# m4drat/wtf

Hardware: AMD Instinct MI355X
Metric: execs/sec + emulated instr/s per node (tlv_server, HEVD) at 1/2/4/8 GPUs (higher is better)
Workload: dtype u64

## Files before the change

### wtf_amd/csrc/engine_run.h

```cpp
#pragma once
#include <hip/hip_runtime.h>

#include "engine_fast.h"

using namespace wtfgpu_dev;

namespace {

__device__ __forceinline__ u64 wave_sum(u64 v) {
#pragma unroll
  for (int off = 32; off > 0; off >>= 1) v += __shfl_xor(v, off, 64);
  return v;
}
__device__ __forceinline__ u64 readlane64(u64 v, int l) {
  const u32 lo = __builtin_amdgcn_readlane((u32)v, l);
  const u32 hi = __builtin_amdgcn_readlane((u32)(v >> 32), l);
  return ((u64)hi << 32) | lo;
}
__device__ __forceinline__ u64 m_eq32(u32 a, u32 b) { return __builtin_amdgcn_uicmp(a, b, 32); }
__device__ __forceinline__ u64 m_ne32(u32 a, u32 b) { return __builtin_amdgcn_uicmp(a, b, 33); }
__device__ __forceinline__ u64 m_eq64(u64 a, u64 b) { return __builtin_amdgcn_uicmpl(a, b, 32); }
__device__ __forceinline__ u64 m_ne64(u64 a, u64 b) { return __builtin_amdgcn_uicmpl(a, b, 33); }
__device__ __forceinline__ u64 m_lt64(u64 a, u64 b) { return __builtin_amdgcn_uicmpl(a, b, 36); }
__device__ __forceinline__ u64 m_ge64(u64 a, u64 b) { return __builtin_amdgcn_uicmpl(a, b, 35); }
__device__ __forceinline__ u64 m_ge32(u32 a, u32 b) { return __builtin_amdgcn_uicmp(a, b, 35); }
__device__ __forceinline__ bool in_mask(u64 m) { return __builtin_amdgcn_inverse_ballot_w64(m); }

__device__ __forceinline__ bool hash_find(const u64 *keys, u32 mask, u64 key, u32 &slot) {
  u32 h = (u32)mix64(key) & mask;
  for (u32 i = 0; i <= mask; i++) {
    const u64 k = rfl64(keys[h]);
    if (k == key) {
      slot = h;
      return true;
    }
    if (k == EMPTY_KEY) return false;
    h = (h + 1) & mask;
  }
  return false;
}

__device__ __forceinline__ bool set_has(const u64 *keys, u32 mask, u64 key) {
  u32 h = (u32)mix64(key) & mask;
  for (u32 i = 0; i <= mask; i++) {
    const u64 k = keys[h];
    if (k == key) return true;
    if (k == EMPTY_KEY) return false;
    h = (h + 1) & mask;
  }
  return false;
}

__device__ __forceinline__ void trace_rip(const Dev &P, u32 lane, u64 rip) {
  const u32 n = P.trace_cnt[lane];
  if (n < P.trace_cap) P.trace[(u64)lane * P.trace_cap + n] = rip;
  P.trace_cnt[lane] = n + 1;
}

__device__ __forceinline__ u64 edge_key(u64 rip, u64 next) {
  u64 e = rip;
  e ^= e >> 30;
  e *= 0xbf58476d1ce4e5b9ull;
  e ^= e >> 27;
  e *= 0x94d049bb133111ebull;
  e ^= e >> 31;
  return e ^ next;
}

__device__ __forceinline__ bool edge_op(u32 op, u32 bsrc) {
  return op == O_JCC || op == O_LOOP || ((op == O_JMP || op == O_CALL) && bsrc != L_IMM);
}

__device__ __forceinline__ void load_lane(const Dev &P, u32 lane, Lane &L) {
  const u64 N = P.nlanes;
#pragma unroll
  for (int i = 0; i < 16; i++) RS(L, i, P.gpr[i * N + lane]);
  L.rip = P.rip[lane];
  L.rflags = P.rflags[lane];
  L.icount = P.icount[lane];
  L.nbytes = P.nbytes[lane];
  L.status = P.status[lane];
  const LaneSys s = P.sys[lane];
  L.cr0 = s.cr0;
  L.cr3 = s.cr3;
  L.efer = s.efer;
  L.cpl = s.cpl;
  L.simd = simd_bits(s.cr0, s.cr4, P.full[lane].xcr0);
  L.ovn = P.ov_count[lane];
  L.lane = lane;
  L.cgen = P.lane_gen ? P.lane_gen[lane] : 0;
  L.ccnt = P.cov_cnt ? P.cov_cnt[lane] : 0;
  if (P.tlb_ok && P.tlb_ok[lane]) {
    const LaneTlb &t = P.tlbs[lane];
#pragma unroll
    for (int i = 0; i < TLB_N; i++) {
      L.tv[i] = t.tv[i];
      L.td[i] = t.td[i];
    }
    L.cvpn = t.cvpn;
    L.cptr = t.cptr;
    L.bloom = t.bloom;
    L.tnext = t.tnext;
  } else {
    L.bloom = 0;
    for (u32 k = 0; k < L.ovn; k++) L.bloom |= bloom_bit(P.ov_gpfn[(u64)k * N + lane]);
    tlb_flush(L);
    L.tnext = 0;
  }
  L.exvec = L.exerr = L.exop = 0;
  L.exaddr = 0;
  L.miss = L.miss_acc = L.flush = L.pend = 0;
  L.nodeliver = 0;
  L.miss_va = 0;
}

__device__ __forceinline__ void store_tlb(const Dev &P, const Lane &L) {
  if (!P.tlb_ok) return;
  LaneTlb &t = P.tlbs[L.lane];
#pragma unroll
  for (int i = 0; i < TLB_N; i++) {
    t.tv[i] = L.tv[i];
    t.td[i] = L.td[i];
  }
  t.cvpn = L.cvpn;
  t.cptr = L.cptr;
  t.bloom = L.bloom;
  t.tnext = L.tnext;
  P.tlb_ok[L.lane] = 1;
}
__device__ __forceinline__ void tlb_stale(const Dev &P, u32 lane) {
  if (P.tlb_ok) P.tlb_ok[lane] = 0;
}

__device__ __forceinline__ void store_lane(const Dev &P, const Lane &L) {
  const u64 N = P.nlanes;
  const u32 lane = L.lane;
#pragma unroll
  for (int i = 0; i < 16; i++) P.gpr[i * N + lane] = R(L, i);
  P.rip[lane] = L.rip;
  P.rflags[lane] = L.rflags;
  P.icount[lane] = L.icount;
  P.nbytes[lane] = L.nbytes;
  P.status[lane] = L.status;
  P.ov_count[lane] = L.ovn;
  if (P.cov_cnt) P.cov_cnt[lane] = L.ccnt;
}

__device__ __forceinline__ u32 log_value(const Dev &P, u64 v, bool mine, u32 lane, u32 gen, u32 cnt);

__device__ __noinline__ u32 cover(const Dev &P, u64 rip, bool mine, u32 lane, u32 gen, u32 cnt) {
  if (P.code_keys) {
    u32 s;
    if (hash_find(P.code_keys, P.code_mask, rip >> 12, s)) {
      const u32 cs = rfl32(P.code_slot[s]);
      if (rfl32(P.cov_map[(u64)cs * WTFGPU_PAGE_SIZE + (rip & 0xfff)])) return cnt;
    } else if (P.extra_keys && set_has(P.extra_keys, P.extra_mask, rip)) {
      return cnt;
    }
  }
  return log_value(P, rip, mine, lane, gen, cnt);
}

__device__ __forceinline__ void count_edge(const Dev &P, u32 lane, bool fresh) {
  if (!P.edge_cnt) return;
  P.edge_cnt[2 * (u64)lane] += 1;
  if (fresh) P.edge_cnt[2 * (u64)lane + 1] += 1;
}

__device__ __noinline__ u32 cover_edge(const Dev &P, u64 e, bool mine, u32 lane, u32 gen, u32 cnt) {
  if (!mine) return cnt;
  if (P.extra_keys && set_has(P.extra_keys, P.extra_mask, e)) return cnt;
  return log_value(P, e, true, lane, gen, cnt);
}

__device__ __forceinline__ u32 log_value(const Dev &P, u64 rip, bool mine, u32 lane, u32 gen, u32 cnt) {
  if (!mine) return cnt;
  const u32 H = P.H;
  const u64 base = (u64)lane * H;
  u32 h = (u32)mix64(rip) & (H - 1);
  for (u32 probe = 0; probe < H; probe++) {
    const u64 idx = base + h;
    if (P.cov_gen[idx] != gen) {
      if (cnt >= H - H / 4) {
        P.cov_overflow[lane] = 1;
        return cnt;
      }
      P.cov_rip[idx] = rip;
      P.cov_gen[idx] = gen;
      return cnt + 1;
    }
    if (P.cov_rip[idx] == rip) return cnt;
    h = (h + 1) & (H - 1);
  }
  return cnt;
}

__device__ __forceinline__ void fetch_bytes(u64 pageptr, u32 off, u32 n, u64 &lo, u64 &hi) {
  const u64 a = (pageptr + off) & ~7ull;
  const u32 sh = (u32)((pageptr + off) & 7);
  const u64 pend = pageptr + WTFGPU_PAGE_SIZE;
  const u64 w0 = rfl64(*(const u64 *)a);
  const u64 w1 = (a + 8 < pend) ? rfl64(*(const u64 *)(a + 8)) : 0;
  const u64 w2 = (a + 16 < pend) ? rfl64(*(const u64 *)(a + 16)) : 0;
  if (sh == 0) {
    lo = w0;
    hi = w1;
  } else {
    lo = (w0 >> (8 * sh)) | (w1 << (64 - 8 * sh));
    hi = (w1 >> (8 * sh)) | (w2 << (64 - 8 * sh));
  }
  if (n < 16) {
    if (n <= 8) {
      hi = 0;
      lo = n == 8 ? lo : (lo & ((1ull << (8 * n)) - 1));
    } else {
      hi &= (1ull << (8 * (n - 8))) - 1;
    }
  }
}

constexpr u32 UC_N = 312;
constexpr u32 UC_U = 4;
constexpr u32 UC_BP = 1, UC_COVERED = 2, UC_CROSS = 4, UC_BADLEN = 8, UC_UNSUP = 16;
struct UCHead {
  u64 key;
  u64 logged;
  u32 flags, pad;
  FOp f;
};
struct UCEntry {
  union {
    UCHead h;
    struct {
      u64 key;
      u64 logged;
      u32 flags, pad;
      FOp f;
    };
  };
  u64 rip;
};
struct UCUop {
  u64 key;
  UOp u;
};
struct GPayload {
  u32 flags, pad;
  FOp f;
  UOp u;
};
constexpr u32 GP_HEAD = (sizeof(u32) * 2 + sizeof(FOp)) / 4;
static_assert(sizeof(UOp) % 4 == 0 && sizeof(FOp) % 4 == 0, "copied as dwords");
static_assert(sizeof(UCEntry) == 64, "LDS entry size");
constexpr u32 UC_QUEUES = 2;
constexpr u64 UC_IMAGE_BYTES = (u64)UC_N * sizeof(UCEntry);

constexpr u32 UC_WAYS = 2;
static_assert(UC_N % UC_WAYS == 0, "whole sets");
__device__ __forceinline__ bool cacheable_key(u64 lptr, u64 pool_lo, u64 pool_span) {
  return !m_ge64(lptr - pool_lo, pool_span);
}
__device__ __forceinline__ u32 uc_slot(u64 key) {
  const u32 h = ((u32)key ^ (u32)(key >> 17)) * 0x9E3779B1u;
  return __umulhi(h, UC_N / UC_WAYS) * UC_WAYS;
}
__device__ __forceinline__ u32 uu_slot(u64 key) { return (u32)((key ^ (key >> 12) * 0x9E3779B1u) & (UC_U - 1)); }

template <typename T>
__device__ __forceinline__ void lds_uniform_read(const T *src, T &dst) {
  const u32 *s = (const u32 *)src;
  u32 *d = (u32 *)&dst;
#pragma unroll
  for (u32 i = 0; i < sizeof(T) / 4; i++) d[i] = rfl32(s[i]);
}

__device__ __forceinline__ void uc_head_read(const UCEntry *e, UCHead &h) {
  h.key = rfl64(e->key);
  h.flags = rfl32(e->flags);
  h.f.w0 = rfl32(e->f.w0);
  h.f.fl = rfl32(e->f.fl);
  h.f.w2 = rfl32(e->f.w2);
  h.f.disp = rfl64(e->f.disp);
  h.f.imm = rfl64(e->f.imm);
}

__device__ __forceinline__ bool bp_lookup(const Dev &P, u64 rip) {
  u32 s;
  return P.bp_keys && hash_find(P.bp_keys, P.bp_mask, rip, s);
}

__device__ __forceinline__ bool lane_phys_write(const Dev &P, Lane &L, u64 gpa, const u8 *src, u64 len) {
  while (len) {
    const u64 off = gpa & 0xfff;
    u64 n = 4096 - off;
    if (n > len) n = len;
    bool priv;
    const u8 *pg = phys_page(P, L.lane, L.ovn, L.bloom, gpa >> 12, priv);
    u8 *dst = (u8 *)pg;
    if (!priv) {
      if (L.ovn >= P.K) return false;
      dst = cow_copy(P, L.lane, L.ovn, gpa >> 12, pg);
      L.ovn++;
      L.bloom |= bloom_bit(gpa >> 12);
    }
    for (u64 i = 0; i < n; i++) dst[off + i] = src[i];
    src += n;
    gpa += n;
    len -= n;
  }
  return true;
}

__device__ __forceinline__ bool lane_phys_write64(const Dev &P, Lane &L, u64 gpa, u64 v) {
  bool priv;
  const u8 *pg = phys_page(P, L.lane, L.ovn, L.bloom, gpa >> 12, priv);
  u8 *dst = (u8 *)pg;
  if (!priv) {
    if (L.ovn >= P.K) return false;
    dst = cow_copy(P, L.lane, L.ovn, gpa >> 12, pg);
    L.ovn++;
    L.bloom |= bloom_bit(gpa >> 12);
  }
  *(u64 *)(dst + (gpa & 0xfff)) = v;
  return true;
}

__device__ __forceinline__ bool has_error_code(u32 vec) {
  return vec == 8 || (vec >= 10 && vec <= 14) || vec == 17 || vec == 21 || vec == 29 || vec == 30;
}
__device__ __forceinline__ bool sup_xlate(const Dev &P, Lane &L, u64 va, int acc, u64 &gpa) {
  u64 td, gpfn;
  if (!walk(P, L, va, acc, td, gpfn)) return false;
  gpa = (gpfn << 12) | (va & 0xfff);
  return true;
}
__device__ __noinline__ bool deliver_fault(const Dev &P, Lane &L) {
  LaneSys &S = P.sys[L.lane];
  const u32 vec = L.exvec, err = L.exerr;
  const u64 cr2 = L.exaddr, frip = L.rip;
  const u32 st0 = L.status, cpl0 = L.cpl;
  bool ok = false;
  do {
    if (S.deliv_icount == L.icount) break;
    if (!S.idtr || vec > 31 || (u64)vec * 16 + 15 > S.idtr_limit) break;
    u64 ga;
    if (!sup_xlate(P, L, S.idtr + vec * 16, ACC_R, ga) || (ga & 0xfff) > 4096 - 16) break;
    bool priv;
    const u8 *g = phys_page(P, L.lane, L.ovn, L.bloom, ga >> 12, priv) + (ga & 0xfff);
    const u64 lo = *(const u64 *)g, hi = *(const u64 *)(g + 8);
    const u32 attr = (u32)(lo >> 40) & 0xff, type = attr & 0xf, ist = (u32)(lo >> 32) & 7;
    if (!(attr & 0x80) || (type != 0xe && type != 0xf)) break;
    const u64 target = (lo & 0xffff) | ((lo >> 32) & 0xffff0000ull) | (hi << 32);
    const u16 sel = (u16)((lo >> 16) & 0xffff);
    const u32 ncpl = sel & 3;
    if (!canonical(target) || ncpl > L.cpl) break;
    u64 rsp = R(L, 4);
    if (ist || ncpl < L.cpl) {
      const u64 off = ist ? 0x24 + (u64)(ist - 1) * 8 : 4 + (u64)ncpl * 8;
      u64 ta;
      if (!sup_xlate(P, L, S.tss + off, ACC_R, ta) || (ta & 0xfff) > 4096 - 8) break;
      const u8 *t = phys_page(P, L.lane, L.ovn, L.bloom, ta >> 12, priv) + (ta & 0xfff);
      u64 v = 0;
      for (int i = 0; i < 8; i++) v |= (u64)t[i] << (8 * i);
      rsp = v;
    }
    rsp &= ~0xfull;
    const bool ec = has_error_code(vec);
    const u32 n = ec ? 6 : 5;
    const u64 ors = R(L, 4), orfl = L.rflags, ocs = S.cs, oss = S.ss;
    L.cpl = 0;
    bool wr = true;
    for (u32 i = 0; i < n && wr; i++) {
      const u32 k = ec ? i : i + 1;
      const u64 w = k == 0 ? (u64)err : k == 1 ? frip : k == 2 ? ocs : k == 3 ? orfl : k == 4 ? ors : oss;
      u64 pa;
      wr = sup_xlate(P, L, rsp - 8 * n + 8 * i, ACC_W, pa) && (pa & 7) == 0 && lane_phys_write64(P, L, pa, w);
    }
    if (!wr) break;
    if (ncpl < cpl0) S.ss = (u16)ncpl;
    set_cs(L, S, sel);
    if (vec == WTFGPU_VEC_PF) S.cr2 = cr2;
    L.cpl = S.cpl = ncpl;
    S.deliv_icount = L.icount;
    RS(L, 4, rsp - 8 * n);
    L.rflags &= ~(0x100ull | 0x4000ull | 0x10000ull | 0x20000ull | (type == 0xe ? 0x200ull : 0));
    L.rip = target;
    L.status = WTFGPU_RUNNING;
    tlb_flush(L);
    L.flush = 0;
    ok = true;
  } while (0);
  if (!ok) {
    L.cpl = cpl0;
    L.status = st0;
    L.exvec = vec;
    L.exerr = err;
    L.exaddr = cr2;
    L.nodeliver = 1;
  }
  return ok;
}

constexpr u32 GUC_WORDS = 48;
constexpr u32 GUC_PAYLOAD = sizeof(GPayload) / 4;
static_assert(GUC_PAYLOAD <= 3 * 14, "global uop cache entry: 3 lines of 14 payload dwords");
__device__ __forceinline__ u32 guc_slot(const Dev &P, u64 key) {
  return (u32)(mix64(key) & P.guc_mask);
}
__device__ __forceinline__ u32 guc_payload_index(u32 lid) {
  return (lid < GUC_WORDS && (lid & 15) < 14) ? (lid >> 4) * 14 + (lid & 15) : ~0u;
}

__device__ __forceinline__ u32 covered_flag(const Dev &P, u64 rip, u32 off) {
  if (P.code_keys) {
    u32 s;
    if (hash_find(P.code_keys, P.code_mask, rip >> 12, s)) {
      const u32 cs = rfl32(P.code_slot[s]);
      if (rfl32(P.cov_map[(u64)cs * WTFGPU_PAGE_SIZE + off])) return UC_COVERED;
    }
  }
  return 0;
}

__device__ __forceinline__ u32 covered_flag_lane(const Dev &P, u64 rip, u32 off) {
  if (!P.code_keys) return 0;
  u32 h = (u32)mix64(rip >> 12) & P.code_mask;
  for (u32 i = 0; i <= P.code_mask; i++) {
    const u64 k = P.code_keys[h];
    if (k == (rip >> 12)) return P.cov_map[(u64)P.code_slot[h] * WTFGPU_PAGE_SIZE + off] ? UC_COVERED : 0;
    if (k == EMPTY_KEY) return 0;
    h = (h + 1) & P.code_mask;
  }
  return 0;
}

__device__ __forceinline__ FOp generic_fop(const UOp &d) {
  FOp f{};
  f.w0 = (d.len & 0x3f) << 20;
  return f;
}

__device__ __forceinline__ bool uc_fill_shared(const Dev &P, UCEntry *e, UCUop *us, u64 key, u32 off, u64 rip,
                                               u32 lid) {
  if (!P.guc) return false;
  const u32 pj = guc_payload_index(lid);
  u32 *head = e ? (u32 *)&e->flags : nullptr, *uop = us ? (u32 *)&us->u : nullptr;
  u32 *gw = P.guc + (u64)guc_slot(P, key) * GUC_WORDS;
  const u32 w = lid < GUC_WORDS ? gw[lid] : 0;
  const bool tag = lid < GUC_WORDS && (lid & 15) >= 14;
  const bool bad = tag && w != ((lid & 1) ? (u32)(key >> 32) : (u32)key);
  if (__ballot(bad) != 0) return false;
  if (pj < GP_HEAD) {
    if (head) head[pj] = w;
  } else if (pj < GUC_PAYLOAD) {
    if (uop) uop[pj - GP_HEAD] = w;
  }
  const u32 sflags = __builtin_amdgcn_readlane(w, 0);
  u32 flags = sflags;
  if (e && !(sflags & UC_COVERED)) {
    flags |= covered_flag(P, rip, off);
    if ((flags & UC_COVERED) && lid == 0) gw[0] = flags;
  }
  __builtin_amdgcn_wave_barrier();
  if (lid == 0) {
    if (us) us->key = key;
    if (e) {
      e->logged = 0;
      e->flags = flags;
      e->rip = rip;
      e->key = key;
    }
  }
  return true;
}

__device__ __noinline__ void uc_fill(const Dev &P, UCEntry *e, UCUop *us, u64 key, u64 lptr, u32 off, u64 rip,
                                     u32 lid, bool shared_checked = false) {
  const u32 pj = guc_payload_index(lid);
  u32 *uop = (u32 *)&us->u;
  if (!shared_checked && uc_fill_shared(P, e, us, key, off, rip, lid)) return;
  u32 *gw = P.guc ? P.guc + (u64)guc_slot(P, key) * GUC_WORDS : nullptr;
  IBytes ib;
  ib.avail = 4096 - off < 16 ? 4096 - off : 16;
  fetch_bytes(lptr, off, ib.avail, ib.lo, ib.hi);
  UOp d;
  const int dr = decode(ib, d);
  u32 flags = dr == 1 ? UC_CROSS : dr == 2 ? UC_BADLEN : 0;
  FOp f;
  if (dr == 0) {
    digest(d, f);
    if (P.edges && edge_op(d.op, d.bsrc)) f = generic_fop(d);
    if (P.trace || g_tn.buf) f = generic_fop(d);
    if (!d.supported) flags |= UC_UNSUP;
    if (bp_lookup(P, rip)) flags |= UC_BP;
  } else {
    f = FOp{};
  }
  const u32 dyn = (dr == 0 && e) ? covered_flag(P, rip, off) : 0;
  if (lid == 0) {
    us->u = d;
    us->key = key;
  }
  __builtin_amdgcn_wave_barrier();
  __builtin_amdgcn_fence(__ATOMIC_RELEASE, "wavefront");
  if (gw) {
    u32 v = 0;
    if (pj < GP_HEAD) v = pj == 0 ? (flags | dyn) : pj == 1 ? 0u : ((const u32 *)&f)[pj - 2];
    else if (pj < GUC_PAYLOAD) v = uop[pj - GP_HEAD];
    else if (lid < GUC_WORDS && (lid & 15) >= 14) v = (lid & 1) ? (u32)(key >> 32) : (u32)key;
    if (lid < GUC_WORDS) gw[lid] = v;
  }
  if (lid == 0 && e) {
    e->logged = 0;
    e->f = f;
    e->flags = flags | dyn;
    e->rip = rip;
    e->key = key;
  }
}

__device__ __forceinline__ const UOp *uc_uop(const Dev &P, UCUop *uu, u64 key, u64 lptr, u32 off, u64 rip, u32 lid) {
  UCUop *us = &uu[uu_slot(key)];
  if (rfl64(us->key) != key) uc_fill(P, nullptr, us, key, lptr, off, rip, lid);
  return &us->u;
}

__device__ __noinline__ void code_xlate(const Dev &P, Lane &L, u64 rip) {
  u64 td;
  const u64 vpn = rip >> 12;
  if (!tlb_get(L, vpn, td) || !perm_ok(L, td, ACC_X)) {
    if (service_miss(P, L, rip & ~0xfffull, ACC_X)) tlb_get(L, vpn, td);
    else td = 0;
    if (td && !perm_ok(L, td, ACC_X)) td = 0;
    if (!td && L.status == WTFGPU_EXIT_FAULT) L.exaddr = rip;
  }
  if (td) {
    L.cvpn = vpn;
    L.cptr = (td & ~0xfffull) | (L.efer & EFER_M32);
  }
}

__device__ __noinline__ bool miss_service(const Dev &P, Lane &L, int attempt) {
  if (attempt >= 16 || !service_miss(P, L, L.miss_va, (int)L.miss_acc)) {
    if (attempt >= 16) set_fault(L, WTFGPU_VEC_GP, 0xffff, L.miss_va);
    return false;
  }
  return true;
}

__device__ __noinline__ int exec_generic(const Dev &P, Lane &L, const UOp *ul, u64 &next) {
  UOp d;
  lds_uniform_read(ul, d);
  return exec(P, L, d, L.rip + d.len, next);
}

__device__ __noinline__ int exec_retry(const Dev &P, Lane &L, const UOp *ul, u64 &next) {
  int x;
  tn_insn_begin(L.lane);
  for (int attempt = 0;; attempt++) {
    L.miss = 0;
    L.pend = 0;
    tn_rollback(L.lane);
    x = exec_generic(P, L, ul, next);
    if (!L.miss || L.status != WTFGPU_RUNNING) break;
    if (!miss_service(P, L, attempt)) break;
  }
  return x;
}

__device__ __forceinline__ void retire(const Dev &P, Lane &L, int x, u32 len, u64 next, u32 opbytes) {
  if (L.flush) {
    tlb_flush(L);
    L.flush = 0;
  }
  if ((x == X_OK || x == X_CR3) && L.status == WTFGPU_RUNNING) {
    L.rip = next;
    L.icount++;
    L.nbytes += len + L.pend;
    if (P.limit && L.icount > P.limit) L.status = WTFGPU_EXIT_TIMEOUT;
    else if (x == X_CR3) L.status = WTFGPU_EXIT_CR3;
  } else if (L.status != WTFGPU_RUNNING) {
  } else if (x == X_UNIMPL) {
    L.status = WTFGPU_EXIT_UNIMPLEMENTED;
    L.exop = len >= 4 ? opbytes : (opbytes & ((1u << (8 * len)) - 1));
  } else if (x == X_INT3) {
    L.status = WTFGPU_EXIT_INT3;
  } else if (x == X_HLT) {
    L.status = WTFGPU_EXIT_HLT;
  }
}

__device__ __noinline__ bool host_write(const Dev &P, Lane &L, u64 va, const u8 *__restrict__ src, u64 n) {
  const u32 cpl0 = L.cpl;
  const u64 cr00 = L.cr0;
  L.cpl = 0;
  L.cr0 &= ~(1ull << 16);
  bool ok = true;
  for (u64 o = 0; o < n;) {
    const u64 a = va + o, room = 4096 - (a & 0xfff);
    const u32 m = (u32)(n - o < room ? n - o : room);
    u8 *d = nullptr;
    u64 td = 0;
    for (int attempt = 0;; attempt++) {
      L.miss = 0;
      if ((d = xlate(L, a, ACC_W, &td))) break;
      if (L.status != WTFGPU_RUNNING || !L.miss || !miss_service(P, L, attempt)) {
        ok = false;
        break;
      }
    }
    if (!ok) break;
    if (td & T_PT) L.flush = 1;
    const u8 *__restrict__ sp = src + o;
    u32 k = 0;
    for (; k + 32 <= m; k += 32) {
      u8 t[32];
#pragma unroll
      for (u32 j = 0; j < 32; j++) t[j] = sp[k + j];
#pragma unroll
      for (u32 j = 0; j < 32; j++) d[k + j] = t[j];
    }
    for (; k < m; k++) d[k] = sp[k];
    o += m;
  }
  if (!ok) {
    if (L.status == WTFGPU_RUNNING || L.status == WTFGPU_EXIT_FAULT) L.status = WTFGPU_EXIT_FEED_FAULT;
    L.miss = 0;
  }
  L.cpl = cpl0;
  L.cr0 = cr00;
  L.pend = 0;
  if (ok && L.flush) {
    tlb_flush(L);
    L.flush = 0;
  }
  return ok;
}

__device__ __noinline__ bool feed_apply(const Dev &P, Lane &L, const wtfgpu_bp_action_t &a) {
  if (!P.feed_pos) return false;
  const u64 pos = P.feed_pos[L.lane];
  if (pos == ~0ull) return false;
  const u64 end = P.feed_end[L.lane];
  if (pos + 4 > end) {
    L.status = WTFGPU_EXIT_STOP_OK;
    return true;
  }
  const u8 *src = P.feed_data + pos;
  const u32 n = (u32)src[0] | ((u32)src[1] << 8) | ((u32)src[2] << 16) | ((u32)src[3] << 24);
  P.feed_pos[L.lane] = pos + 4 + n;
  if (n >= a.value || pos + 4 + n > end) {
    L.status = WTFGPU_EXIT_STOP_OK;
    return true;
  }
  const u32 rb = (u32)a.gprs[0] & 15, rn = (u32)a.gprs[1] & 15;
  const u64 dst = R(L, rb) + a.value - n;
  if (!host_write(P, L, dst, src + 4, n)) return true;
  RS(L, rn, n);
  RS(L, rb, dst);
  return true;
}

__device__ __noinline__ void insert_apply(const Dev &P, Lane &L, const wtfgpu_insert_t &ins) {
  const u64 pos = P.feed_pos[L.lane], end = P.feed_end[L.lane];
  if (pos == ~0ull) return;
  P.feed_pos[L.lane] = end;
  if (pos + 8 > end) return;
  const u8 *src = P.feed_data + pos;
  const u32 n = (u32)src[0] | ((u32)src[1] << 8) | ((u32)src[2] << 16) | ((u32)src[3] << 24);
  if (n < 4 || pos + 4 + n > end) return;
  const u32 head = (u32)src[4] | ((u32)src[5] << 8) | ((u32)src[6] << 16) | ((u32)src[7] << 24);
  const u64 m = n - 4;
  RS(L, ins.head_reg & 15, head);
  if (!host_write(P, L, R(L, ins.ptr_reg & 15), src + 8, m)) return;
  RS(L, ins.len_reg & 15, m);
  if (ins.len_arg) {
    u8 le[8];
    for (int i = 0; i < 8; i++) le[i] = (u8)(m >> (8 * i));
    host_write(P, L, R(L, WTFGPU_RSP) + 8 + 8 * (u64)ins.len_arg, le, 8);
  }
}

__device__ __forceinline__ u32 rotr32(u32 x, u32 n) { return (x >> n) | (x << (32 - n)); }
__device__ __forceinline__ void b3_g(u32 *v, int a, int b, int c, int d, u32 x, u32 y) {
  v[a] = v[a] + v[b] + x;
  v[d] = rotr32(v[d] ^ v[a], 16);
  v[c] = v[c] + v[d];
  v[b] = rotr32(v[b] ^ v[c], 12);
  v[a] = v[a] + v[b] + y;
  v[d] = rotr32(v[d] ^ v[a], 8);
  v[c] = v[c] + v[d];
  v[b] = rotr32(v[b] ^ v[c], 7);
}
__device__ __noinline__ void blake3_le64(u64 in, u64 &lo, u64 &hi) {
  const u32 iv[8] = {0x6A09E667u, 0xBB67AE85u, 0x3C6EF372u, 0xA54FF53Au,
                     0x510E527Fu, 0x9B05688Cu, 0x1F83D9ABu, 0x5BE0CD19u};
  const u8 perm[16] = {2, 6, 3, 10, 7, 0, 4, 13, 1, 11, 12, 5, 9, 14, 15, 8};
  u32 m[16] = {(u32)in, (u32)(in >> 32), 0, 0, 0, 0, 0, 0, 0, 0, 0, 0, 0, 0, 0, 0};
  u32 v[16] = {iv[0], iv[1], iv[2], iv[3], iv[4], iv[5], iv[6], iv[7], iv[0], iv[1], iv[2], iv[3], 0, 0, 8, 1 | 2 | 8};
  for (int r = 0; r < 7; r++) {
    b3_g(v, 0, 4, 8, 12, m[0], m[1]);
    b3_g(v, 1, 5, 9, 13, m[2], m[3]);
    b3_g(v, 2, 6, 10, 14, m[4], m[5]);
    b3_g(v, 3, 7, 11, 15, m[6], m[7]);
    b3_g(v, 0, 5, 10, 15, m[8], m[9]);
    b3_g(v, 1, 6, 11, 12, m[10], m[11]);
    b3_g(v, 2, 7, 8, 13, m[12], m[13]);
    b3_g(v, 3, 4, 9, 14, m[14], m[15]);
    if (r < 6) {
      u32 t[16];
      for (int i = 0; i < 16; i++) t[i] = m[perm[i]];
      for (int i = 0; i < 16; i++) m[i] = t[i];
    }
  }
  lo = (u64)(v[0] ^ v[8]) | ((u64)(v[1] ^ v[9]) << 32);
  hi = (u64)(v[2] ^ v[10]) | ((u64)(v[3] ^ v[11]) << 32);
}

__device__ __forceinline__ bool bp_apply_action(const Dev &P, Lane &L, u64 grip, const wtfgpu_bp_action_t *found) {
  u32 s;
  if (!found && (!P.act_keys || !hash_find(P.act_keys, P.act_mask, grip, s))) return false;
  const wtfgpu_bp_action_t &a = found ? *found : P.act[s];
  if (a.kind == WTFGPU_BPACT_SET_GPRS) {
    for (u32 i = 0; i < 16; i++) RS(L, i, a.gprs[i]);
    L.rip = a.gprs[16];
    return true;
  }
  if (a.kind == WTFGPU_BPACT_FEED) return feed_apply(P, L, a);
  if (a.kind == WTFGPU_BPACT_STOP_OK) {
    L.status = WTFGPU_EXIT_STOP_OK;
    return true;
  }
  if (a.kind == WTFGPU_BPACT_RDRAND) {
    if (!P.rd_seed) return false;
    u64 lo, hi;
    blake3_le64(P.rd_seed[L.lane], lo, hi);
    P.rd_seed[L.lane] = lo;
    RS(L, (u32)a.gprs[0] & 15, hi);
    return true;
  }
  if (a.kind == WTFGPU_BPACT_STOP_ARGS) {
    if (!P.stop_args) return false;
    const u64 rsp = R(L, WTFGPU_RSP);
    u64 v[6] = {R(L, 1), R(L, 2), R(L, 8), R(L, 9), 0, 0};
    for (u32 i = 4; i < 6 && i < a.value; i++) {
      for (int attempt = 0;; attempt++) {
        L.miss = 0;
        if (vread(L, rsp + 8 + 8 * (u64)i, 8, v[i])) break;
        if (L.status != WTFGPU_RUNNING || !L.miss || !miss_service(P, L, attempt)) {
          L.status = WTFGPU_RUNNING;
          L.miss = 0;
          L.pend = 0;
          return false;
        }
      }
    }
    L.pend = 0;
    for (u32 i = 0; i < 6; i++) P.stop_args[(u64)L.lane * 6 + i] = i < a.value ? v[i] : 0;
    L.status = WTFGPU_EXIT_STOP_ARGS;
    return true;
  }
  if (a.kind != WTFGPU_BPACT_RETURN) return false;
  if (a.gprs[0]) {
    const u64 s = R(L, (u32)(a.gprs[0] - 1) & 15);
    const u64 lim = a.gprs[1];
    for (u64 i = 0; i < lim;) {
      const u64 va = s + i, al = va & ~31ull;
      const u8 *p = nullptr;
      for (int attempt = 0;; attempt++) {
        L.miss = 0;
        if ((p = xlate(L, al, ACC_R))) break;
        if (L.status != WTFGPU_RUNNING || !L.miss || !miss_service(P, L, attempt)) {
          L.status = WTFGPU_RUNNING;
          L.miss = 0;
          return false;
        }
      }
      const u64 *w = (const u64 *)p;
      const u64 c0 = w[0], c1 = w[1], c2 = w[2], c3 = w[3];
      bool term = false;
      for (u32 b = (u32)(va - al); b < 32 && i < lim && !term; b++, i++) {
        const u64 c = b < 8 ? c0 : b < 16 ? c1 : b < 24 ? c2 : c3;
        term = ((c >> (8 * (b & 7))) & 0xff) == 0;
      }
      if (term) break;
    }
  }
  const u64 rsp = R(L, WTFGPU_RSP);
  u64 ra = 0;
  for (int attempt = 0;; attempt++) {
    L.miss = 0;
    if (vread(L, rsp, 8, ra)) break;
    if (L.status != WTFGPU_RUNNING || !L.miss || !miss_service(P, L, attempt)) {
      L.status = WTFGPU_RUNNING;
      L.miss = 0;
      L.pend = 0;
      return false;
    }
  }
  L.pend = 0;
  RS(L, WTFGPU_RAX, a.value);
  RS(L, WTFGPU_RSP, rsp + 8);
  L.rip = ra;
  return true;
}

__device__ __noinline__ bool bp_apply(const Dev &P, Lane &L, u64 grip, const wtfgpu_bp_action_t *found = nullptr) {
  tn_mute(L.lane);
  const bool r = bp_apply_action(P, L, grip, found);
  tn_unmute(L.lane, 0, 0, 0, false);
  return r;
}

__device__ __noinline__ void slow_step(const Dev &P, Lane &L, u64 grip, u64 lptr, bool ing, bool &skip) {
  const u32 off = (u32)(grip & 0xfff);
  const bool m32 = (lptr & EFER_M32) != 0;
  lptr &= ~EFER_M32;
  IBytes ib;
  ib.avail = 4096 - off < 16 ? 4096 - off : 16;
  fetch_bytes(lptr, off, ib.avail, ib.lo, ib.hi);
  UOp d;
  int dr = decode(ib, d, m32);
  if (dr == 1) {
    u64 nptr = 0;
    if (ing) {
      const u64 va2 = (grip & ~0xfffull) + 4096;
      u64 td;
      if (!tlb_get(L, va2 >> 12, td) || !perm_ok(L, td, ACC_X)) {
        if (service_miss(P, L, va2, ACC_X)) tlb_get(L, va2 >> 12, td);
        else td = 0;
      }
      if (td) nptr = td & ~0xfffull;
      else ing = false;
    }
    const u64 cm = __ballot(ing);
    if (cm == 0) return;
    const int leader = __ffsll((long long)cm) - 1;
    const u64 lnptr = readlane64(nptr, leader);
    ing = ing && nptr == lnptr;
    const u32 n0 = ib.avail;
    u64 lo2, hi2;
    fetch_bytes(lnptr, 0, 16 - n0, lo2, hi2);
    if (n0 >= 8) {
      ib.hi = (n0 == 8 ? 0 : ib.hi) | (n0 == 8 ? lo2 : (lo2 << (8 * (n0 - 8))));
    } else {
      ib.lo = ib.lo | (lo2 << (8 * n0));
      ib.hi = (lo2 >> (64 - 8 * n0)) | (hi2 << (8 * n0));
    }
    ib.avail = 16;
    dr = decode(ib, d, m32);
  }
  if (dr == 2) {
    if (ing) set_fault(L, WTFGPU_VEC_GP, 0, 0);
    return;
  }
  const u64 gmask = __ballot(ing);
  if (gmask == 0) return;
  if (P.cov_rip) L.ccnt = cover(P, grip, ing, L.lane, L.cgen, L.ccnt);
  if (P.trace && ing && !skip) trace_rip(P, L.lane, grip);
  const bool isbp = bp_lookup(P, grip);
  if (ing) {
    if (isbp && !skip) {
      const bool applied = bp_apply(P, L, grip);
      if (!applied) L.status = WTFGPU_EXIT_BREAKPOINT;
      skip = applied && L.rip == grip;
      if (applied && !skip && g_tn.buf) tn_regs(P, L);
      ing = false;
    } else {
      skip = false;
    }
  }
  if (!d.supported) {
    if (ing) {
      L.status = WTFGPU_EXIT_UNIMPLEMENTED;
      L.exop = d.len >= 4 ? d.opbytes : (d.opbytes & ((1u << (8 * d.len)) - 1));
    }
    return;
  }
  if (ing) {
    u64 next = 0;
    int x;
    tn_insn_begin(L.lane);
    for (int attempt = 0;; attempt++) {
      L.miss = 0;
      L.pend = 0;
      tn_rollback(L.lane);
      x = exec(P, L, d, grip + d.len, next);
      if (!L.miss || L.status != WTFGPU_RUNNING) break;
      if (!miss_service(P, L, attempt)) break;
    }
    retire(P, L, x, d.len, next, d.opbytes);
    if (g_tn.buf && (x == X_OK || x == X_CR3)) tn_regs(P, L);
    if (P.edges && P.cov_rip && edge_op(d.op, d.bsrc) && x == X_OK) {
      const u32 c0 = L.ccnt;
      L.ccnt = cover_edge(P, edge_key(grip, next), true, L.lane, L.cgen, L.ccnt);
      count_edge(P, L.lane, L.ccnt != c0);
    }
  }
}

struct LaneCopy {
  Lane l;
  u32 r[32];
};
#define WITH_LANE_COPY(call)                      \
  do {                                            \
    LaneCopy &C_ = ((LaneCopy *)P.lcopy)[lane];   \
    Lane &T = C_.l;                               \
    u32 *const tlo_ = C_.r, *const thi_ = C_.r + 16; \
    _Pragma("unroll") for (int i_ = 0; i_ < 16; i_++) { \
      tlo_[i_] = glo[i_];                         \
      thi_[i_] = ghi[i_];                         \
    }                                             \
    T = L;                                        \
    T.glo = tlo_;                                 \
    T.ghi = thi_;                                 \
    call;                                         \
    L = T;                                        \
    L.glo = glo;                                  \
    L.ghi = ghi;                                  \
    _Pragma("unroll") for (int i_ = 0; i_ < 16; i_++) { \
      glo[i_] = tlo_[i_];                         \
      ghi[i_] = thi_[i_];                         \
    }                                             \
  } while (0)

#ifdef WTFGPU_STAMPS
#define STAMP(k)                                   \
  do {                                             \
    const u64 t_ = __builtin_amdgcn_s_memtime();   \
    stamp_[k] += t_ - tprev_;                      \
    tprev_ = t_;                                   \
  } while (0)
#define WHY(k) why_ = (k)
#define OPHIST(op) ophist_[((op) & 63) | (why_ & 3) << 6 | ((op) & 64 ? 256 : 0)]++
constexpr u32 STAT_N = 536;
#else
constexpr u32 STAT_N = 16;
#define OPHIST(op) \
  do {             \
  } while (0)
#define STAMP(k) \
  do {           \
  } while (0)
#define WHY(k) \
  do {         \
  } while (0)
#endif

#define RECONVERGE() __builtin_amdgcn_wave_barrier()

constexpr u32 FILL_PREFETCH = 8;
__global__ __launch_bounds__(256, 2) void k_run(Dev P, u32 first, u32 count, u64 max_steps) {
  if (P.perm && rfl64(P.stat[3]) == 0) return;
  const u32 lid = threadIdx.x & 63;
  const u32 hw = rfl32(blockIdx.x * 4 + (threadIdx.x >> 6));
  const u32 tid = hw * P.lpw + lid;
  const bool inrange = lid < P.lpw && tid < count && first + tid < P.nlanes;
  const u32 lane = inrange ? (P.perm ? P.perm[first + tid] : first + tid) : 0;
  const bool valid = inrange && P.status[lane] == WTFGPU_RUNNING;
  __shared__ UCEntry sUC[4][UC_N];
  __shared__ UCUop sUU[4][UC_U];
  UCEntry *uc = sUC[threadIdx.x >> 6];
  UCUop *uu = sUU[threadIdx.x >> 6];
  const bool wave_live = __ballot(valid) != 0;
  const UCEntry *img = (P.warm && wave_live) ? (const UCEntry *)P.warm + (u64)(hw % P.warm_n) * UC_N : nullptr;
  if (img) {
    for (u32 i = lid; i < UC_N; i += 64) {
      UCEntry t = img[i];
      t.logged = 0;
      if (P.cov_rip && t.key != EMPTY_KEY && !(t.flags & (UC_COVERED | UC_CROSS | UC_BADLEN)))
        t.flags |= covered_flag_lane(P, t.rip, (u32)(t.rip & 0xfff));
      uc[i] = t;
    }
  } else {
    for (u32 i = lid; i < UC_N; i += 64) uc[i].key = EMPTY_KEY;
  }
  if (lid < UC_U) uu[lid].key = EMPTY_KEY;
  u32 glo[16], ghi[16];
  Lane L;
  L.glo = glo;
  L.ghi = ghi;
  if (valid) {
    load_lane(P, lane, L);
  } else {
    L.status = WTFGPU_EXIT_IDLE;
    L.lane = 0;
    L.rip = 0;
    L.icount = 0;
    L.cvpn = EMPTY_KEY;
  }
  const u64 icount0 = L.icount;
  bool skip = valid && (P.lflags[lane] & 1);
  if (valid && g_tn.buf && (g_tn.pos[lane] == 0 || (P.lflags[lane] & 2))) WITH_LANE_COPY(tn_regs(P, T));
  const bool cov_on = rfl32(P.cov_rip != nullptr ? 1u : 0u) != 0;
  u64 pool_lo = (u64)(uintptr_t)P.pool, pool_span = (P.npool + 1) * WTFGPU_PAGE_SIZE;
  u64 limit_v = P.limit ? P.limit : ~0ull;
  u32 max32 = max_steps > 0xffffffffull ? 0xffffffffu : (u32)max_steps;
  asm volatile("" : "+v"(pool_lo), "+v"(pool_span), "+v"(limit_v), "+v"(max32));
  const FastMem fm = fast_mem(P);
  u32 steps = 0;
#ifdef WTFGPU_STAMPS
  u64 stamp_[8] = {0, 0, 0, 0, 0, 0, 0, 0};
  u64 tprev_ = __builtin_amdgcn_s_memtime();
  u64 whyc_[4] = {0, 0, 0, 0};
  u32 why_ = 3;
  u32 ophist_[512] = {};
  u64 bpcyc_[8] = {};
#endif

  for (;;) {
    u64 grip = 0;
    bool have = false;
    for (;;) {
      if (m_ge32(steps, max32)) break;
      const u64 am = m_eq32(L.status, WTFGPU_RUNNING);
      if (am == 0) break;
      grip = readlane64(L.rip, __ffsll((long long)am) - 1);
      u64 gm = am & m_eq64(L.rip, grip);
      if (gm != am) {
        for (u64 lo = am & m_lt64(L.rip, grip); lo; lo = am & m_lt64(L.rip, grip))
          grip = readlane64(L.rip, __ffsll((long long)lo) - 1);
        gm = am & m_eq64(L.rip, grip);
      }
      have = true;
      WHY(1);
      if (const u64 cxm = gm & m_ne64(L.cvpn, grip >> 12)) {
        if (in_mask(cxm)) {
          u64 td, gp;
          bool ok = tlb_get(L, grip >> 12, td) && perm_ok(L, td, ACC_X);
          if (!ok && walk<false>(P, L, grip & ~0xfffull, ACC_X, td, gp) && perm_ok(L, td, ACC_X)) {
            tlb_put(L, grip >> 12, td);
            ok = true;
          }
          if (ok) {
            L.cvpn = grip >> 12;
            L.cptr = (td & ~0xfffull) | (L.efer & EFER_M32);
          }
        }
        if (gm & m_ne64(L.cvpn, grip >> 12)) break;
      }
      WHY(3);
      const u64 lptr = readlane64(L.cptr, __ffsll((long long)gm) - 1);
      if (m_ge64(lptr - pool_lo, pool_span)) break;
      const u64 ingm = gm & m_eq64(L.cptr, lptr);
      const bool ing = in_mask(ingm);
      const u64 key = lptr | (grip & 0xfff);
      UCEntry *e = &uc[uc_slot(key)];
      UCHead h;
      uc_head_read(e, h);
      if (h.key != key) uc_head_read(++e, h);
      WHY(2);
      if (h.key != key) break;
      WHY(3);
      const u32 flags = h.flags;
      if (flags & (UC_CROSS | UC_BADLEN | UC_UNSUP)) break;
      if ((flags & UC_BP) && (ingm & ~__ballot(skip))) break;
      if (cov_on && !(flags & UC_COVERED) && (ingm & ~rfl64(e->logged))) break;
      const FOp &f = h.f;
      if (fo_op(f) == FO_GENERIC) break;
      if (!(f.fl & (FF_PUSH | FF_POP | FF_MR_A | FF_MR_B | FF_MW)) && fo_op(f) < FO_VLD) {
        steps++;
        have = false;
        if (ing) {
          skip = false;
          const u32 len = fo_len(f);
          FOp fr = f;
          asm volatile("" : "+s"(fr.w0), "+s"(fr.fl), "+s"(fr.w2), "+s"(fr.disp), "+s"(fr.imm));
          u64 next;
          fast_exec<true>(fm, L, fr, grip + len, next);
          L.rip = next;
          L.icount++;
          L.nbytes += len;
          if (L.icount > limit_v) L.status = WTFGPU_EXIT_TIMEOUT;
        }
        RECONVERGE();
        continue;
      }
      steps++;
      have = false;
      STAMP(6);
      const u32 len = fo_len(f);
      u64 next = 0;
      u64 wantm = ingm;
      if (ing) skip = false;
      for (u32 round = 0;; round++) {
        if (in_mask(wantm)) {
          L.miss = 0;
          L.pend = 0;
          FOp fr = f;
          asm volatile("" : "+s"(fr.w0), "+s"(fr.fl), "+s"(fr.w2), "+s"(fr.disp), "+s"(fr.imm));
          fast_exec(fm, L, fr, grip + len, next);
        }
        RECONVERGE();
        wantm = round >= 3 ? 0 : wantm & m_eq32(L.miss, 2);
        if (wantm == 0) break;
        u64 csrc = 0, cdst = 0, cgpfn = 0, ctd = 0;
        bool want = in_mask(wantm);
        if (want && !fast_fill_prep(P, L, csrc, cdst, cgpfn, ctd)) {
          want = false;
          fast_fault(P, L);
        }
        for (u64 cm = __ballot(want && cdst); cm; cm &= cm - 1) {
          const int l = __ffsll((long long)cm) - 1;
          const uint4 *s4 = (const uint4 *)(uintptr_t)readlane64(csrc, l) + lid * 4;
          uint4 *d4 = (uint4 *)(uintptr_t)readlane64(cdst, l) + lid * 4;
          const uint4 a = s4[0], b = s4[1], c = s4[2], d = s4[3];
          d4[0] = a;
          d4[1] = b;
          d4[2] = c;
          d4[3] = d;
        }
        __builtin_amdgcn_fence(__ATOMIC_ACQ_REL, "workgroup");
        if (want && cdst) fast_fill_finish(P, L, cdst, cgpfn, ctd);
        wantm = __ballot(want);
      }
      const u64 missm = ingm & m_ne32(L.miss, 0);
      if (in_mask(ingm & ~missm)) {
        L.rip = next;
        L.icount++;
        L.nbytes += len + L.pend;
        if (L.icount > limit_v) L.status = WTFGPU_EXIT_TIMEOUT;
      }
      RECONVERGE();
      STAMP(7);
      if (missm & m_eq32(L.status, WTFGPU_RUNNING)) {
        WHY(0);
        steps--;
        have = true;
        break;
      }
      if (missm) break;
    }
    STAMP(0);
    if (__ballot(L.status == WTFGPU_EXIT_FAULT && !L.nodeliver)) {
      if (L.status == WTFGPU_EXIT_FAULT && !L.nodeliver) {
        bool dv;
        WITH_LANE_COPY(dv = deliver_fault(P, T));
        if (dv && g_tn.buf) WITH_LANE_COPY(tn_regs(P, T));
      }
      RECONVERGE();
      continue;
    }
    if (!have) break;

    steps++;
#ifdef WTFGPU_STAMPS
    whyc_[why_ & 3]++;
#endif
    const bool active = L.status == WTFGPU_RUNNING;
    bool cand = active && L.rip == grip;
    if (cand && (grip >> 12) != L.cvpn) WITH_LANE_COPY(code_xlate(P, T, grip));
    cand = cand && (grip >> 12) == L.cvpn;
    const u64 cm = __ballot(cand);
    if (cm == 0) continue;
    const int leader = __ffsll((long long)cm) - 1;
    const u64 lptr = readlane64(L.cptr, leader);
    bool ing = cand && L.cptr == lptr;

    const u32 off = (u32)(grip & 0xfff);
    const u64 key = lptr | off;
    UCEntry *e = &uc[uc_slot(key)];
    if (rfl64(e->key) != key) {
      if (rfl64(e[1].key) == key) e += 1;
      else if (cacheable_key(lptr, pool_lo, pool_span)) {
        if (lid < 16) ((u32 *)&e[1])[lid] = ((const u32 *)e)[lid];
        __builtin_amdgcn_wave_barrier();
      }
    }
    const bool cacheable = !m_ge64(lptr - pool_lo, pool_span);
    if (cacheable && rfl64(e->key) != key) {
      if (!uc_fill_shared(P, e, &uu[uu_slot(key)], key, off, grip, lid))
        uc_fill(P, e, &uu[uu_slot(key)], key, lptr, off, grip, lid, true);
      const UCEntry *pe = e;
      u64 prip = grip;
      for (u32 k = 0; k < FILL_PREFETCH; k++) {
        const u32 pf = rfl32(pe->flags), pw0 = rfl32(pe->f.w0), plen = (pw0 >> 20) & 0x3f;
        if ((pf & (UC_CROSS | UC_BADLEN)) || !plen) break;
        const u64 nxt = prip + plen;
        if ((nxt >> 12) != (grip >> 12) || (nxt & 0xfff) > 4096 - 16) break;
        const u32 poff = (u32)(nxt & 0xfff);
        const u64 pkey = lptr | poff;
        UCEntry *ps = &uc[uc_slot(pkey)];
        if (rfl64(ps->key) == pkey || rfl64(ps[1].key) == pkey) break;
        if (!uc_fill_shared(P, ps + 1, nullptr, pkey, poff, nxt, lid)) break;
        pe = ps + 1;
        prip = nxt;
      }
      const u32 ff = rfl32(e->flags);
      if (!(ff & (UC_BP | UC_CROSS | UC_BADLEN | UC_UNSUP)) && (!cov_on || (ff & UC_COVERED)) &&
          (rfl32(e->f.w0) & 0xff) != FO_GENERIC) {
        steps--;
        STAMP(2);
        continue;
      }
    }
    STAMP(2);
    const u32 flags = cacheable ? rfl32(e->flags) : UC_CROSS;
    if (flags & (UC_CROSS | UC_BADLEN)) {
      if (flags & UC_BADLEN) {
        if (ing) set_fault(L, WTFGPU_VEC_GP, 0, 0);
      } else if (L.status != WTFGPU_EXIT_IDLE) {
        bool sk = skip;
        WITH_LANE_COPY(slow_step(P, T, grip, lptr, ing, sk));
        skip = sk;
      }
      RECONVERGE();
      STAMP(5);
      continue;
    }
    const u32 len = (rfl32(e->f.w0) >> 20) & 0x3f;
    const u64 gmask = __ballot(ing);

    if (P.trace && ing && !skip) trace_rip(P, L.lane, grip);
    bool logged_now = false;
    if (cov_on && !(flags & UC_COVERED)) {
      const u64 logged = rfl64(e->logged);
      if (gmask & ~logged) {
        L.ccnt = cover(P, grip, ing && !((logged >> lid) & 1), L.lane, L.cgen, L.ccnt);
        if (lid == 0) e->logged = logged | gmask;
        logged_now = true;
      }
    }
    STAMP(3);
    if (logged_now && !(flags & (UC_BP | UC_UNSUP)) && (rfl32(e->f.w0) & 0xff) != FO_GENERIC) {
      steps--;
      continue;
    }
    u32 act_kind = ~0u;
    const wtfgpu_bp_action_t *act = nullptr;
    if ((flags & UC_BP) && P.act_keys && !g_tn.buf) {
      u32 slot;
      if (hash_find(P.act_keys, P.act_mask, grip, slot)) {
        act = &P.act[slot];
        act_kind = rfl32(act->kind);
      }
    }
#ifdef WTFGPU_STAMPS
    if (__ballot(ing && (flags & UC_BP) && !skip)) OPHIST(56 + (act_kind < 7 ? act_kind : 7));
#endif
    if (act_kind == WTFGPU_BPACT_SET_GPRS && ing && !skip) {
#pragma unroll
      for (u32 i = 0; i < 16; i++) RS(L, i, act->gprs[i]);
      L.rip = act->gprs[16];
      skip = L.rip == grip;
      ing = false;
    }
    if (act_kind == WTFGPU_BPACT_STOP_OK && ing && !skip) {
      L.status = WTFGPU_EXIT_STOP_OK;
      skip = true;
      ing = false;
    }
    if (act_kind == WTFGPU_BPACT_FEED && P.feed_pos) {
      bool want = false;
      if (ing && !skip) {
        const u64 pos = P.feed_pos[L.lane];
        const u64 end = P.feed_end[L.lane];
        if (pos != ~0ull && pos + 4 <= end) {
          const u8 *src = P.feed_data + pos;
          const u32 n = (u32)src[0] | ((u32)src[1] << 8) | ((u32)src[2] << 16) | ((u32)src[3] << 24);
          const u64 win = act->value;
          if (n && n < win && pos + 4 + n <= end) {
            const u64 va = R(L, (u32)act->gprs[0] & 15) + win - n;
            u64 td;
            if (!(tlb_get(L, va >> 12, td) && (td & T_PRIV))) {
              L.miss_va = va;
              L.miss_acc = ACC_W;
              want = true;
            }
          }
        }
      }
      u64 csrc = 0, cdst = 0, cgpfn = 0, ctd = 0;
      if (want) {
        const u32 cpl0 = L.cpl;
        const u64 cr00 = L.cr0;
        L.cpl = 0;
        L.cr0 &= ~(1ull << 16);
        want = fast_fill_prep(P, L, csrc, cdst, cgpfn, ctd);
        L.cpl = cpl0;
        L.cr0 = cr00;
      }
      RECONVERGE();
      for (u64 cm = __ballot(want && cdst); cm; cm &= cm - 1) {
        const int l = __ffsll((long long)cm) - 1;
        const uint4 *s4 = (const uint4 *)(uintptr_t)readlane64(csrc, l) + lid * 4;
        uint4 *d4 = (uint4 *)(uintptr_t)readlane64(cdst, l) + lid * 4;
        const uint4 a = s4[0], b = s4[1], c = s4[2], d = s4[3];
        d4[0] = a;
        d4[1] = b;
        d4[2] = c;
        d4[3] = d;
      }
      __builtin_amdgcn_fence(__ATOMIC_ACQ_REL, "workgroup");
      if (want && cdst) fast_fill_finish(P, L, cdst, cgpfn, ctd);
      RECONVERGE();
    }
    if (ing) {
      if ((flags & UC_BP) && !skip) {
        bool applied = false;
#ifdef WTFGPU_STAMPS
        const u64 tb_ = __builtin_amdgcn_s_memtime();
#endif
        if (P.act_keys) WITH_LANE_COPY(applied = bp_apply(P, T, grip, act));
#ifdef WTFGPU_STAMPS
        bpcyc_[act_kind < 7 ? act_kind : 7] += __builtin_amdgcn_s_memtime() - tb_;
#endif
        if (!applied) L.status = WTFGPU_EXIT_BREAKPOINT;
        skip = applied && L.rip == grip;
        if (applied && !skip && g_tn.buf) WITH_LANE_COPY(tn_regs(P, T));
        ing = false;
      } else {
        skip = false;
      }
    }
    STAMP(4);
    const UOp *u = nullptr;
    if (__ballot(ing)) u = uc_uop(P, uu, key, lptr, off, grip, lid);
    if (__ballot(ing) && !(flags & UC_UNSUP)) OPHIST(rfl32(u->op) + (flags & UC_COVERED ? 64 : 0));
    if (ing && (flags & UC_UNSUP)) {
      const u32 ob = u->opbytes, n = len;
      L.status = WTFGPU_EXIT_UNIMPLEMENTED;
      L.exop = n >= 4 ? ob : (ob & ((1u << (8 * n)) - 1));
      ing = false;
    }
    if (ing) {
      u64 next = 0;
      int x;
      WITH_LANE_COPY(x = exec_retry(P, T, u, next));
      u32 opbytes = 0;
      if (x == X_UNIMPL) opbytes = u->opbytes;
      retire(P, L, x, len, next, opbytes);
      if (g_tn.buf && (x == X_OK || x == X_CR3)) WITH_LANE_COPY(tn_regs(P, T));
      if (P.edges && P.cov_rip && x == X_OK && edge_op(rfl32(u->op), rfl32(u->bsrc))) {
        const u32 c0 = L.ccnt;
        L.ccnt = cover_edge(P, edge_key(grip, next), true, L.lane, L.cgen, L.ccnt);
        count_edge(P, L.lane, L.ccnt != c0);
      }
    }
    RECONVERGE();
    STAMP(1);
  }

  if (P.warm && wave_live && hw < P.warm_n) {
    __builtin_amdgcn_wave_barrier();
    __builtin_amdgcn_fence(__ATOMIC_ACQUIRE, "wavefront");
    UCEntry *out = (UCEntry *)P.warm + (u64)hw * UC_N;
    for (u32 i = lid; i < UC_N; i += 64) out[i] = uc[i];
  }
  if (valid && g_tn.buf && L.status != WTFGPU_RUNNING && L.status != WTFGPU_EXIT_BREAKPOINT &&
      g_tn.pos[lane] > g_tn.ipos[lane])
    WITH_LANE_COPY(tn_regs(P, T));
  if (valid) {
    store_lane(P, L);
    store_tlb(P, L);
    if (L.status == WTFGPU_EXIT_FAULT || L.status == WTFGPU_EXIT_UNIMPLEMENTED) {
      ExitInfo ei;
      ei.vector = L.exvec;
      ei.error = L.exerr;
      ei.opcode = L.exop;
      ei.cpl = L.cpl;
      ei.addr = L.exaddr;
      P.exinfo[lane] = ei;
    }
    P.lflags[lane] = skip ? 1u : 0u;
  }
  const u64 retired = wave_sum(valid ? L.icount - icount0 : 0);
  const u64 running = wave_sum((valid && L.status == WTFGPU_RUNNING) ? 1 : 0);
  if (lid == 0) {
    atomicAdd((unsigned long long *)&P.stat[0], (unsigned long long)steps);
    atomicAdd((unsigned long long *)&P.stat[1], (unsigned long long)retired);
    if (running) atomicAdd((unsigned long long *)&P.stat[2], (unsigned long long)running);
#ifdef WTFGPU_STAMPS
    for (int k = 0; k < 8; k++) atomicAdd((unsigned long long *)&P.stat[4 + k], (unsigned long long)stamp_[k]);
    for (int k = 0; k < 4; k++) atomicAdd((unsigned long long *)&P.stat[12 + k], (unsigned long long)whyc_[k]);
    for (int k = 0; k < 512; k++)
      if (ophist_[k]) atomicAdd((unsigned long long *)&P.stat[16 + k], (unsigned long long)ophist_[k]);
    for (int k = 0; k < 8; k++) atomicAdd((unsigned long long *)&P.stat[528 + k], (unsigned long long)bpcyc_[k]);
#endif
  }
}

}
```

Measured before the change: 15.66 million.

## Prefetch following decoded instructions in parallel across lanes from global uop cache

```diff
diff --git a/wtf_amd/csrc/engine_run.h b/wtf_amd/csrc/engine_run.h
--- a/wtf_amd/csrc/engine_run.h
+++ b/wtf_amd/csrc/engine_run.h
@@ -411,6 +411,20 @@
   return (lid < GUC_WORDS && (lid & 15) < 14) ? (lid >> 4) * 14 + (lid & 15) : ~0u;
 }
 
+__device__ __forceinline__ u32 guc_head_sum(u64 key, u32 flags, u32 w0, u32 fl, u32 w2, u64 disp, u64 imm) {
+  u32 h = ((u32)key ^ 0x811C9DC5u) * 0x01000193u;
+  h = (h ^ (u32)(key >> 32)) * 0x01000193u;
+  h = (h ^ (flags & ~UC_COVERED)) * 0x01000193u;
+  h = (h ^ w0) * 0x01000193u;
+  h = (h ^ fl) * 0x01000193u;
+  h = (h ^ w2) * 0x01000193u;
+  h = (h ^ (u32)disp) * 0x01000193u;
+  h = (h ^ (u32)(disp >> 32)) * 0x01000193u;
+  h = (h ^ (u32)imm) * 0x01000193u;
+  h = (h ^ (u32)(imm >> 32)) * 0x01000193u;
+  return h ^ (h >> 15);
+}
+
 __device__ __forceinline__ u32 covered_flag(const Dev &P, u64 rip, u32 off) {
   if (P.code_keys) {
     u32 s;
@@ -505,7 +519,10 @@
   __builtin_amdgcn_fence(__ATOMIC_RELEASE, "wavefront");
   if (gw) {
     u32 v = 0;
-    if (pj < GP_HEAD) v = pj == 0 ? (flags | dyn) : pj == 1 ? 0u : ((const u32 *)&f)[pj - 2];
+    if (pj < GP_HEAD)
+      v = pj == 0   ? (flags | dyn)
+          : pj == 1 ? guc_head_sum(key, flags, f.w0, f.fl, f.w2, f.disp, f.imm)
+                    : ((const u32 *)&f)[pj - 2];
     else if (pj < GUC_PAYLOAD) v = uop[pj - GP_HEAD];
     else if (lid < GUC_WORDS && (lid & 15) >= 14) v = (lid & 1) ? (u32)(key >> 32) : (u32)key;
     if (lid < GUC_WORDS) gw[lid] = v;
@@ -517,6 +534,75 @@
     e->rip = rip;
     e->key = key;
   }
+}
+
+constexpr u32 FILL_WINDOW = 32;
+static_assert(FILL_WINDOW <= 64, "one candidate offset per lane");
+__device__ __forceinline__ void uc_fill_window(const Dev &P, UCEntry *uc, const UCEntry *e, u64 lptr, u64 grip,
+                                               u32 lid) {
+  if (!P.guc) return;
+  __builtin_amdgcn_wave_barrier();
+  __builtin_amdgcn_fence(__ATOMIC_ACQ_REL, "wavefront");
+  const u32 pf = rfl32(e->flags), plen = (rfl32(e->f.w0) >> 20) & 0x3f;
+  if ((pf & (UC_CROSS | UC_BADLEN)) || !plen) return;
+  const u32 off0 = (u32)(grip & 0xfff) + plen;
+  if (off0 > 4096 - 16) return;
+  const u64 key0 = lptr | off0;
+  const UCEntry *s0 = &uc[uc_slot(key0)];
+  if (rfl64(s0->key) == key0 || rfl64(s0[1].key) == key0) return;
+  const u32 poff = off0 + lid;
+  const bool probe = lid < FILL_WINDOW && poff <= 4096 - 16;
+  const u64 pkey = lptr | poff;
+  u32 *gw = P.guc + (u64)guc_slot(P, pkey) * GUC_WORDS;
+  uint4 a = {0, 0, 0, 0}, b = {0, 0, 0, 0};
+  uint2 c = {0, 0}, t0 = {0, 0}, t1 = {0, 0}, t2 = {0, 0};
+  if (probe) {
+    a = *(const uint4 *)gw;
+    b = *(const uint4 *)(gw + 4);
+    c = *(const uint2 *)(gw + 8);
+    t0 = *(const uint2 *)(gw + 14);
+    t1 = *(const uint2 *)(gw + 30);
+    t2 = *(const uint2 *)(gw + 46);
+  }
+  const u32 klo = (u32)pkey, khi = (u32)(pkey >> 32);
+  const u32 flags = a.x, len = (a.z >> 20) & 0x3f;
+  const u64 disp = b.z | ((u64)b.w << 32), imm = c.x | ((u64)c.y << 32);
+  bool ok = probe && t0.x == klo && t0.y == khi && t1.x == klo && t1.y == khi && t2.x == klo && t2.y == khi &&
+            a.y == guc_head_sum(pkey, flags, a.z, a.w, b.x, disp, imm) && !(flags & (UC_CROSS | UC_BADLEN)) &&
+            len != 0;
+  const u32 set = probe ? uc_slot(pkey) : 0;
+  if (ok) ok = uc[set].key != pkey && uc[set + 1].key != pkey;
+  const u64 okm = __ballot(ok);
+  u64 chain = 0, lose = 0;
+  for (u32 pos = 0; pos < FILL_WINDOW && ((okm >> pos) & 1);) {
+    chain |= 1ull << pos;
+    const u32 ps = __builtin_amdgcn_readlane(set, pos);
+    lose |= __ballot(set == ps) & ~((2ull << pos) - 1);
+    pos += __builtin_amdgcn_readlane(len, pos);
+  }
+  if (((chain & ~lose) >> lid) & 1) {
+    const u64 prip = (grip & ~0xfffull) | poff;
+    u32 fl = flags;
+    if (!(fl & UC_COVERED)) {
+      fl |= covered_flag_lane(P, prip, poff);
+      if (fl & UC_COVERED) gw[0] = fl;
+    }
+    UCEntry *d = &uc[set + 1];
+    d->logged = 0;
+    d->flags = fl;
+    d->pad = a.y;
+    d->f.w0 = a.z;
+    d->f.fl = a.w;
+    d->f.w2 = b.x;
+    d->f.pad = b.y;
+    d->f.disp = disp;
+    d->f.imm = imm;
+    d->rip = prip;
+    __builtin_amdgcn_fence(__ATOMIC_RELEASE, "wavefront");
+    d->key = pkey;
+  }
+  __builtin_amdgcn_wave_barrier();
+  __builtin_amdgcn_fence(__ATOMIC_ACQ_REL, "wavefront");
 }
 
 __device__ __forceinline__ const UOp *uc_uop(const Dev &P, UCUop *uu, u64 key, u64 lptr, u32 off, u64 rip, u32 lid) {
@@ -950,7 +1036,6 @@
 
 #define RECONVERGE() __builtin_amdgcn_wave_barrier()
 
-constexpr u32 FILL_PREFETCH = 8;
 __global__ __launch_bounds__(256, 2) void k_run(Dev P, u32 first, u32 count, u64 max_steps) {
   if (P.perm && rfl64(P.stat[3]) == 0) return;
   const u32 lid = threadIdx.x & 63;
@@ -1172,21 +1257,7 @@
     if (cacheable && rfl64(e->key) != key) {
       if (!uc_fill_shared(P, e, &uu[uu_slot(key)], key, off, grip, lid))
         uc_fill(P, e, &uu[uu_slot(key)], key, lptr, off, grip, lid, true);
-      const UCEntry *pe = e;
-      u64 prip = grip;
-      for (u32 k = 0; k < FILL_PREFETCH; k++) {
-        const u32 pf = rfl32(pe->flags), pw0 = rfl32(pe->f.w0), plen = (pw0 >> 20) & 0x3f;
-        if ((pf & (UC_CROSS | UC_BADLEN)) || !plen) break;
-        const u64 nxt = prip + plen;
-        if ((nxt >> 12) != (grip >> 12) || (nxt & 0xfff) > 4096 - 16) break;
-        const u32 poff = (u32)(nxt & 0xfff);
-        const u64 pkey = lptr | poff;
-        UCEntry *ps = &uc[uc_slot(pkey)];
-        if (rfl64(ps->key) == pkey || rfl64(ps[1].key) == pkey) break;
-        if (!uc_fill_shared(P, ps + 1, nullptr, pkey, poff, nxt, lid)) break;
-        pe = ps + 1;
-        prip = nxt;
-      }
+      uc_fill_window(P, uc, e, lptr, grip, lid);
       const u32 ff = rfl32(e->flags);
       if (!(ff & (UC_BP | UC_CROSS | UC_BADLEN | UC_UNSUP)) && (!cov_on || (ff & UC_COVERED)) &&
           (rfl32(e->f.w0) & 0xff) != FO_GENERIC) {
```

Result: no change. 15.52 million (-0.9%).
